# M-Gjerde/GaussianSplattingViewer

Measured on AMD Instinct MI355X. Metric: frames/sec + Msplats/sec, 1M Gaussians @ 1920×1080, 1/2/4/8 MI355X, higher is better.
Workload: dtype f32

## Files before the change

gaussiansplattingviewer_amd/csrc/api.hip:

```cpp
#include <algorithm>
#include <chrono>
#include <cstdio>
#include <cstdlib>
#include <cstring>
#include <mutex>
#include <string>
#include <vector>

#include "gsr.h"
#include "gsr_internal.h"

namespace {

thread_local std::string g_err;

int fail(int code, const std::string &msg) {
    g_err = msg;
    return code;
}

#define GSR_HIP(call, what)                                                                  \
    do {                                                                                     \
        hipError_t e_ = (call);                                                              \
        if (e_ != hipSuccess)                                                                \
// ... 70 lines not shown
    Buf<uint32_t> block_kept{bufs};
    Buf<uint32_t> color_ids{bufs};
    Buf<uint32_t> perm{bufs};
    Buf<uint32_t> ds_ctl{bufs};
    Buf<uint32_t> col_hist{bufs};
    Buf<uint32_t> tile_keys{bufs}, tile_vals{bufs}, tile_keys_alt{bufs}, tile_vals_alt{bufs};
    Buf<uint2> ranges_local{bufs};
    uint32_t *ranges_words() const { return reinterpret_cast<uint32_t *>(ranges_local.get()); }
    Buf<uint32_t> col_starts{bufs};
    Buf<uint32_t> blend_order{bufs};
    Buf<float> grad2d{bufs};
    Buf<int32_t> bwd_radii{bufs};
    Buf<float> cam_partials{bufs};
    Buf<uint64_t> det_slab{bufs}, det_partials{bufs};
    Buf<float> det_sums{bufs};
    Buf<uint8_t> det_marks{bufs};
    hipEvent_t ev_bwd[4] = {};
    bool bwd_timed = false;
    Buf<uint32_t> frame_words{bufs};
    uint32_t *list_n() const { return frame_words.get() + 1; }
    GsrHostWords *host_words = nullptr, *d_host_words = nullptr;
    uint32_t sort_tag = 0;
    uint32_t last_Dr = UINT32_MAX, last_D = UINT32_MAX;
    struct LastFrame {
        bool valid = false;
        int64_t K = 0;
        int64_t list = 0;
        bool tight = false;
        uint32_t gx = 0, gy = 0, rb = 0, re = 0;
        uint32_t *point_list = nullptr, *tiles_local = nullptr;
        bool packed = false;
        uint32_t id_mask = 0xFFFFFFFFu;
    } last;
    int cull = 1;
    int fast = 1;
    int depth_sort = -1;
    int tight = 1;
    int timing = 0;
    int64_t forwards = 0;
    int64_t timed_frames = 0;
    hipEvent_t ev[kTimingRing][kStages + 1] = {};
    hipEvent_t ev_color[kTimingRing][2] = {};
    int second_stream = 1;
    hipStream_t aux = nullptr;
    hipEvent_t fork = nullptr, join = nullptr;
    hipEvent_t compacted = nullptr;
    int graphs = 0;
    uint32_t ws_gen = 0;
    int64_t list_cap = 0;
    std::vector<GraphEntry> graph_cache;
    std::vector<hipGraphExec_t> graph_retired;
    uint64_t graph_clock = 0;
    int64_t graph_frames = 0, graph_records = 0, graph_overflows = 0;
};

namespace {

int order_stream(gsr_context *ctx, hipStream_t s) {
    if (ctx->ws_stream_set && s != ctx->ws_stream)
        GSR_HIP(hipDeviceSynchronize(), "hipDeviceSynchronize(stream switch)");
    ctx->ws_stream = s;
    ctx->ws_stream_set = true;
    return GSR_OK;
}

int grow(gsr_context *ctx, DevBuf &b, size_t bytes, hipStream_t s) {
// ... 60 lines not shown
}

template <typename Pred>
bool spin_on(const unsigned long long *word, Pred pred, uint64_t &value) {
    const auto t0 = std::chrono::steady_clock::now();
    for (uint32_t spin = 0;; ++spin) {
        value = __atomic_load_n(word, __ATOMIC_ACQUIRE);
        if (pred(value)) return true;
        if ((spin & 1023u) == 1023u && std::chrono::steady_clock::now() - t0 > kSpinLimit)
            return false;
    }
}

uint64_t host_word(const unsigned long long &word) {
    return __atomic_load_n(&word, __ATOMIC_ACQUIRE);
}

struct Frame {
    hipStream_t s;
    int64_t P;
    int W, H;
    uint32_t gx, gy, rb, re, rows_tiles;
    int y0, rows_out;
    uint64_t T_strip;
    bool dbg;
    int tmode;
    hipEvent_t *ev, *evc;
    bool compact_sort;
    bool msd_sort;
    bool main_publish;
    bool color_ids;
    bool colpairs;
    bool graph = false;
    int col_shift;
    uint32_t tag;
    bool wide_local;
    GsrPreprocessArgs pa;
    bool tight;
    int shading = GSR_SHADE_SPLAT;
    float *depth_map = nullptr, *inv_depth_map = nullptr;
    float *median_depth = nullptr;
    int32_t *median_id = nullptr;
    int feat_C = 0;
    const float *features = nullptr;
    float *feature_map = nullptr;
    bool no_blend = false;
    uint64_t K = 0;
    uint64_t KL = 0;
    uint32_t *point_list = nullptr, *tiles_local = nullptr;
    uint32_t id_mask = 0xFFFFFFFFu;
};

struct FrameRequest {
    int shading = GSR_SHADE_SPLAT;
    const gsr_depth_outputs *depth = nullptr;
    const gsr_surface_outputs *surface = nullptr;
    bool antialiasing = false;
    bool no_blend = false;
    const gsr_feature_outputs *feat = nullptr;
};

int stage_end(gsr_context *ctx, const Frame &f, int i) {
    if (f.tmode == 1 || (f.tmode == 2 && i >= 5))
        GSR_HIP(hipEventRecord(f.ev[i + 1], f.s), "hipEventRecord");
    if (f.dbg) {
        GSR_HIP(hipStreamSynchronize(f.s), std::string("stage ") + kStageNames[i]);
// ... 45 lines not shown
        f.feat_C = rq.feat->C, f.features = rq.feat->features, f.feature_map = rq.feat->feature_map;
    f.no_blend = rq.no_blend;
    f.P = P;
    f.W = W;
    f.H = H;
    f.gx = (uint32_t)((W + GSR_TILE_X - 1) / GSR_TILE_X);
    f.gy = (uint32_t)((H + GSR_TILE_Y - 1) / GSR_TILE_Y);
    if (f.gx > 0xFFFFu || f.gy > 0xFFFFu)
        return fail(GSR_E_INVALID, "gsr_forward: image larger than 65535 tiles per side");
    f.rb = 0;
    f.re = f.gy;
    if (st->tile_row_begin != 0 || st->tile_row_end != 0) {
        if (st->tile_row_begin < 0 || st->tile_row_end > (int)f.gy ||
            st->tile_row_begin >= st->tile_row_end)
            return fail(GSR_E_INVALID, "gsr_forward: bad tile row strip");
        f.rb = (uint32_t)st->tile_row_begin;
        f.re = (uint32_t)st->tile_row_end;
    }
    f.rows_tiles = f.re - f.rb;
    f.y0 = (int)(f.rb * GSR_TILE_Y);
    f.rows_out = std::min(H, (int)(f.re * GSR_TILE_Y)) - f.y0;
    f.T_strip = (uint64_t)f.gx * f.rows_tiles;
    f.dbg = st->debug != 0;
    f.ev = ctx->ev[ctx->timed_frames % kTimingRing];
    f.evc = ctx->ev_color[ctx->timed_frames % kTimingRing];
    f.tmode = ctx->timing == 1 ? 1 : (ctx->timing == 2 && ctx->forwards++ % 8 == 0) ? 2 : 0;

    const int ybits = f.rows_tiles > 1 ? bits_for(f.rows_tiles - 1) : 0;
    f.col_shift = 32 - ybits;
    f.colpairs = f.gx <= 256 && f.rows_tiles <= 256 &&
                 (f.col_shift == 32 || (uint64_t)P <= (1ull << f.col_shift));

    GSR_TRY(reserve_P(ctx, P, s));
    GSR_TRY(grow(ctx, ctx->ranges_local, (size_t)std::max<uint64_t>(f.T_strip, 1) * 8, s));
    if (f.colpairs) {
        GSR_TRY(grow(ctx, ctx->col_starts, 257 * 4, s));
        GSR_TRY(grow(ctx, ctx->blend_order,
                     (size_t)gsr_blend_order_groups((uint32_t)f.T_strip) * 4, s));
    }

    GsrPreprocessArgs &pa = f.pa;
    pa = GsrPreprocessArgs{};
    pa.P = P;
    pa.D = g->D;
    pa.M = g->M;
    pa.scale_modifier = g->scale_modifier;
    pa.means3D = g->means3D;
    pa.scales = g->scales;
    pa.rotations = g->rotations;
    pa.opacities = g->opacities;
    pa.shs = g->shs;
    pa.colors_precomp = g->colors_precomp;
    pa.cov3D_precomp = g->cov3D_precomp;
    pa.viewmatrix = st->viewmatrix;
    pa.projmatrix = st->projmatrix;
    pa.campos = st->campos;
    pa.tanfovx = st->tanfovx;
    pa.tanfovy = st->tanfovy;
    pa.focal_y = (float)H / (2.0f * st->tanfovy);
    pa.focal_x = (float)W / (2.0f * st->tanfovx);
    pa.W = W;
    pa.H = H;
    pa.grid_x = f.gx;
    pa.grid_y = f.gy;
    pa.row_begin = f.rb;
    pa.row_end = f.re;
    pa.prefiltered = st->prefiltered;
// ... 4 lines not shown
    pa.strip_skip = out->radii == nullptr ? 1 : 0;
    pa.records = ctx->records.get();
    pa.sort_keys = ctx->sort_keys.get();
    f.compact_sort = ctx->depth_sort < 0 ? (f.rows_tiles < f.gy && P >= kCompactP)
                                         : ctx->depth_sort == 1 || ctx->depth_sort == 3;
    pa.block_kept = f.compact_sort ? ctx->block_kept.get() : nullptr;
    f.msd_sort = ctx->depth_sort < 0
                     ? ctx->last_Dr <= (ctx->second_stream ? kMsdMaxD : kMsdMaxDOneStream)
                     : ctx->depth_sort >= 2;
    f.main_publish = f.msd_sort && !f.compact_sort;
    pa.strip_rect = ctx->strip_rect.get();
    f.tight = ctx->tight && f.colpairs && !out->n_contrib && f.rows_tiles == f.gy &&
              rq.shading != GSR_SHADE_BILLBOARD;
    pa.strip_rc = f.tight ? ctx->strip_rc.get() : nullptr;
    pa.block_pairs = ctx->pair_count.get();
    pa.host_words = ctx->d_host_words;
    pa.depths = out->depths;
    pa.means2D = out->means2D;
    pa.conic_opacity = out->conic_opacity;
    pa.rgb = out->rgb;
    pa.tiles_touched = out->tiles_touched;
    f.color_ids = f.compact_sort && gsr_color_ids_ok(pa);
    if (f.color_ids) GSR_TRY(grow(ctx, ctx->color_ids, (size_t)P * 4, s));
    f.tag = ++ctx->sort_tag;
    if (f.tag == 0) f.tag = ++ctx->sort_tag;
    pa.k_tag = f.tag;
    {
        const uint32_t crowd = (uint32_t)host_word(ctx->host_words->crowd);
        f.wide_local = crowd != 0u && f.tag - crowd <= kCrowdFrames;
    }
    return GSR_OK;
}

int launch_depth_sort(gsr_context *ctx, const Frame &f, int p0, int p1) {
    uint32_t *hist = ctx->hist.get(), *digit_total = ctx->digit_total.get();
    uint32_t *ctl = ctx->ds_ctl.get(), *perm = ctx->perm.get();
    uint2 *ds_a = ctx->ds_a.get(), *ds_b = ctx->ds_b.get();
    unsigned long long *host_D = &ctx->d_host_words->sort_D;
    hipError_t e;
    const int64_t nb = gsr_preprocess_blocks(f.P);
    const uint2 *keybits = reinterpret_cast<const uint2 *>(f.pa.block_pairs + nb);
    if (f.compact_sort) {
        if (f.msd_sort && p0 != 0) return GSR_OK;
        uint32_t *keys_c = ctx->ds_b_words(), *ids_c = keys_c + f.P;
        e = gsr_depth_sort_compacted(f.pa.sort_keys, f.P, f.pa.block_kept, keys_c, ids_c, ds_a,
                                     ds_b, perm, hist, digit_total, ctl, p0, p1, f.s, host_D,
                                     f.tag, f.color_ids ? ctx->color_ids.get() : nullptr,
                                     f.color_ids ? ctx->compacted : nullptr, f.msd_sort ? 1 : 0,
                                     f.msd_sort && !f.main_publish ? keybits : nullptr, nb);
    } else if (f.msd_sort) {
        if (p0 != 0) return GSR_OK;
        e = gsr_depth_sort_msd(f.pa.sort_keys, f.P, f.main_publish ? nullptr : keybits, nb,
                               ds_a, ds_b, perm, hist, digit_total, ctl, f.s,
                               f.graph ? nullptr : host_D, f.tag,
                               f.graph ? nullptr : &ctx->d_host_words->crowd,
                               f.graph ? 0 : f.wide_local);
    } else {
        e = gsr_depth_sort(f.pa.sort_keys, f.P, 1, ds_a, ds_b, perm, hist, digit_total, ctl, p0,
                           p1, f.s, f.graph ? nullptr : host_D, f.tag);
    }
    GSR_HIP(e, "depth sort launch");
    return GSR_OK;
}

constexpr int kColorWavesFull = 2, kColorWavesCompacted = 3, kColorWavesStrip = 4;
int color_waves_of(const Frame &f) {
// ... 107 lines not shown
                                       std::to_string(ctx->last_D) + ", sort " +
                                       std::to_string(ctl2[1]) + ")");
        if (!f.colpairs && scan_K[0] != f.K)
            return fail(GSR_E_HIP, "gsr_forward: pair count mismatch (preprocess " +
                                       std::to_string(f.K) + ", scan " +
                                       std::to_string(scan_K[0]) + ")");
    }
    int64_t want = (int64_t)f.KL;
    if (ctx->graphs && f.colpairs && want > ctx->list_cap) {
        ctx->list_cap = list_capacity(want, ctx->list_cap);
        want = ctx->list_cap;
    }
    return reserve_K(ctx, want, f.s);
}

uint32_t id_mask_of(int col_shift) {
    return col_shift < 32 ? (1u << col_shift) - 1u : 0xFFFFFFFFu;
}

int launch_col_binning(gsr_context *ctx, Frame &f, int64_t n, uint32_t *list_n) {
    uint32_t *tv = ctx->tile_vals.get(), *tv_alt = ctx->tile_vals_alt.get();
    uint32_t *col_starts = ctx->col_starts.get();
    if (n > 0)
        GSR_HIP(gsr_launch_col_pairs_scatter(ctx->perm.get(), ctx->rect_sorted.get(),
                                             f.tight ? ctx->rc_sorted.get() : nullptr, f.P,
                                             ctx->ds_ctl.get(), ctx->col_hist.get(),
                                             ctx->digit_total.get(), f.col_shift, tv_alt,
                                             col_starts, f.s,
                                             list_n ? (uint32_t)n : 0xFFFFFFFFu, list_n),
                "column scatter launch");
    std::swap(tv, tv_alt);
    GSR_TRY(stage_end(ctx, f, 3));
    const GsrTileStarts ts{col_starts, f.gx, f.rows_tiles, ctx->ranges_local.get(),
                           ctx->blend_order.get()};
    if (n > 0 && f.col_shift < 32)
        GSR_HIP(gsr_radix_sort_keys(&tv, &tv_alt, n, f.col_shift, 32, ctx->hist.get(),
                                    ctx->digit_total.get(), f.s, list_n, &ts),
                "tile sort launch");
    else
        GSR_HIP(gsr_launch_tile_runs(n, list_n, ts, f.s), "tile ranges launch");
    GSR_TRY(stage_end(ctx, f, 4));
    f.point_list = tv;
    f.tiles_local = nullptr;
    f.id_mask = id_mask_of(f.col_shift);
    return GSR_OK;
}

int launch_binning(gsr_context *ctx, Frame &f) {
    const int64_t K = (int64_t)f.KL;
    if (f.colpairs) return launch_col_binning(ctx, f, K, nullptr);
    const uint32_t *perm = ctx->perm.get(), *d_valid = ctx->ds_ctl.get();
    uint32_t *hist = ctx->hist.get(), *digit_total = ctx->digit_total.get();
    uint32_t *tk = ctx->tile_keys.get(), *tv = ctx->tile_vals.get();
    uint32_t *tk_alt = ctx->tile_keys_alt.get(), *tv_alt = ctx->tile_vals_alt.get();
    const int tbits = f.T_strip > 1 ? bits_for(f.T_strip - 1) : 0;
    const GsrRadixPlan plan = gsr_radix_plan(0, tbits);
    if (K > 0) {
        GSR_HIP(gsr_launch_scan_down(perm, ctx->rect_sorted.get(), ctx->partials.get(), f.P,
                                     d_valid, ctx->total.get(), ctx->bin.get(),
                                     ctx->chunk_first.get(), f.s),
                "scan_down launch");
        GSR_HIP(gsr_launch_dup_sort_pass(ctx->bin.get(), ctx->chunk_first.get(), K, f.gx,
                                         plan.n ? plan.shift[0] : 0, plan.n ? plan.nbits[0] : 0,
                                         hist, digit_total, tk_alt, tv_alt,
                                         ctx->ranges_local.get(), (uint32_t)f.T_strip, f.s),
                "duplicate launch");
        std::swap(tk, tk_alt);
// ... 51 lines not shown
    } else if (f.depth_map || f.inv_depth_map) {
        const GsrDepthArgs da{f.pa.sort_keys, f.depth_map, f.inv_depth_map};
        GSR_HIP(gsr_launch_blend_depth(ba, da, f.s), "depth blend launch");
    } else {
        GSR_HIP(gsr_launch_blend(ba, f.s), "blend launch");
    }
    if (f.feature_map)
        GSR_HIP(gsr_launch_blend_features(ba, f.features, f.feat_C, f.feature_map, f.s),
                "feature blend launch");
    return GSR_OK;
}

struct JoinGuard {
    hipStream_t s = nullptr;
    hipEvent_t join = nullptr;
    bool armed = false;
    ~JoinGuard() {
        if (armed) (void)hipStreamWaitEvent(s, join, 0);
    }
};

void finish_frame(gsr_context *ctx, const Frame &f, gsr_outputs *out) {
    out->num_rendered = (int64_t)f.K;
    gsr_context::LastFrame &l = ctx->last;
    l.K = (int64_t)f.K;
    l.list = (int64_t)f.KL;
    l.tight = f.tight;
    l.gx = f.gx, l.gy = f.gy, l.rb = f.rb, l.re = f.re;
    l.point_list = f.point_list;
    l.tiles_local = f.tiles_local;
    l.id_mask = f.id_mask;
    l.packed = f.colpairs && f.KL > 0;
    l.valid = true;
    if (f.tmode) ++ctx->timed_frames;
}

int frame_head(gsr_context *ctx, const Frame &f) {
    if (f.tmode == 1) GSR_HIP(hipEventRecord(f.ev[0], f.s), "hipEventRecord");
    GSR_HIP(gsr_launch_preprocess(f.pa, f.s), "preprocess launch");
    GSR_HIP(hipEventRecord(ctx->fork, f.s), "hipEventRecord(fork)");
    return stage_end(ctx, f, 0);
}

int frame_tail(gsr_context *ctx, const Frame &f, const gsr_raster_settings *st,
               gsr_outputs *out) {
    if (ctx->second_stream)
        GSR_HIP(hipStreamWaitEvent(f.s, ctx->join, 0), "hipStreamWaitEvent(join)");
    GSR_TRY(stage_end(ctx, f, 5));
    if (!f.no_blend) GSR_TRY(launch_blend(ctx, f, st, out));
    return stage_end(ctx, f, 6);
}


bool graph_eligible(const gsr_context *ctx, const Frame &f, const gsr_outputs *out) {
    return ctx->graphs && ctx->list_cap > 0 && f.colpairs && !f.dbg && f.tmode != 1 &&
           !f.compact_sort && !f.color_ids && !out->rgb && f.P > 0;
}

GraphKey graph_key(const gsr_context *ctx, const Frame &f) {
    GraphKey k;
    std::memset(&k, 0, sizeof(k));
    k.ws_gen = ctx->ws_gen;
    k.cap = ctx->list_cap;
    k.P = f.P;
    k.means3D = f.pa.means3D;
    k.shs = f.pa.shs;
    k.colors_precomp = f.pa.colors_precomp;
    k.D = f.pa.D;
    k.M = f.pa.M;
    k.W = f.W;
    k.H = f.H;
    k.gx = f.gx;
    k.gy = f.gy;
    k.rb = f.rb;
    k.re = f.re;
    k.col_shift = f.col_shift;
    k.color_waves = color_waves_of(f);
    k.msd = f.msd_sort;
    k.main_publish = f.main_publish;
    k.tight = f.tight;
    k.sh_vec4 = (uint8_t)f.pa.sh_vec4;
    return k;
}

GsrPreprocessArgs graph_args(const gsr_context *ctx, const GsrPreprocessArgs &a) {
    GsrPreprocessArgs g = a;
    g.campos = a.campos ? reinterpret_cast<const float *>(ctx->frame_words.get() + 4) : nullptr;
    g.viewmatrix = g.projmatrix = nullptr;
    g.scales = g.rotations = g.opacities = g.cov3D_precomp = nullptr;
    g.radii = nullptr;
    g.depths = g.means2D = g.conic_opacity = g.rgb = nullptr;
    g.tiles_touched = nullptr;
    g.k_tag = 0;
    g.frame_words = nullptr;
    return g;
}

void retire_graph(gsr_context *ctx, GraphEntry &e) {
    for (hipGraphExec_t *ge : {&e.sort, &e.bin, &e.aux}) {
        if (*ge) ctx->graph_retired.push_back(*ge);
        *ge = nullptr;
    }
}

int drain_retired(gsr_context *ctx, hipStream_t s, bool force) {
    if (ctx->graph_retired.empty() || (!force && ctx->graph_retired.size() < kGraphRetired))
        return GSR_OK;
    GSR_HIP(hipStreamSynchronize(s), "hipStreamSynchronize(graphs)");
    if (ctx->aux) GSR_HIP(hipStreamSynchronize(ctx->aux), "hipStreamSynchronize(graphs)");
    for (hipGraphExec_t ge : ctx->graph_retired) (void)hipGraphExecDestroy(ge);
    ctx->graph_retired.clear();
    return GSR_OK;
}

struct CaptureStream {
    hipStream_t s = nullptr;
    bool own = false;
    ~CaptureStream() {
        if (own && s) (void)hipStreamDestroy(s);
    }
};

template <typename Chain>
int record_chain(gsr_context *ctx, Chain chain, hipGraphExec_t *out) {
    CaptureStream capture;
    capture.s = ctx->aux;
    if (!capture.s) {
// ... 10 lines not shown
        if (graph) (void)hipGraphDestroy(graph);
        return rc;
    }
    GSR_HIP(e, "hipStreamEndCapture");
    const hipError_t ei = hipGraphInstantiate(out, graph, nullptr, nullptr, 0);
    (void)hipGraphDestroy(graph);
    GSR_HIP(ei, "hipGraphInstantiate");
    return GSR_OK;
}

Frame graph_frame(const gsr_context *ctx, const Frame &f) {
    Frame g = f;
    g.pa = graph_args(ctx, f.pa);
    g.tmode = 0;
    return g;
}

int chain_sort(gsr_context *ctx, Frame &g, hipStream_t cs) {
    g.s = cs;
    if (g.main_publish)
        GSR_HIP(gsr_launch_count_pairs(g.pa, cs, ctx->ds_ctl.get(), ctx->frame_words.get()),
                "pair count launch");
    return launch_depth_sort(ctx, g, 0, gsr_depth_sort_passes(32));
}

int chain_bin(gsr_context *ctx, Frame &g, hipStream_t cs) {
    g.s = cs;
    GSR_TRY(launch_scan(ctx, g));
    return launch_col_binning(ctx, g, ctx->list_cap, ctx->list_n());
}

int record_frame_graphs(gsr_context *ctx, const Frame &f, GraphEntry &e) {
    Frame g = graph_frame(ctx, f);
    const uint32_t *fw = ctx->frame_words.get();
    GSR_TRY(record_chain(ctx, [&](hipStream_t cs) { return chain_sort(ctx, g, cs); }, &e.sort));
    GSR_TRY(record_chain(ctx, [&](hipStream_t cs) { return chain_bin(ctx, g, cs); }, &e.bin));
    e.point_list = g.point_list;
    GSR_TRY(record_chain(ctx, [&](hipStream_t cs) { return aux_chain(ctx, g, cs, fw); }, &e.aux));
    ++ctx->graph_records;
    return GSR_OK;
}

int find_graphs(gsr_context *ctx, const Frame &f, GraphEntry **out) {
    const GraphKey key = graph_key(ctx, f);
    GraphEntry *hit = nullptr;
    for (auto it = ctx->graph_cache.begin(); it != ctx->graph_cache.end();) {
        if (it->key.ws_gen != ctx->ws_gen || it->key.cap != ctx->list_cap) {
            retire_graph(ctx, *it);
            it = ctx->graph_cache.erase(it);
            continue;
        }
        if (std::memcmp(&it->key, &key, sizeof(key)) == 0) hit = &*it;
        ++it;
    }
    if (!hit) {
        if (ctx->graph_cache.size() >= kGraphCache) {
            auto lru = std::min_element(ctx->graph_cache.begin(), ctx->graph_cache.end(),
                                        [](const GraphEntry &a, const GraphEntry &b) {
                                            return a.used < b.used;
                                        });
            retire_graph(ctx, *lru);
            ctx->graph_cache.erase(lru);
        }
        GraphEntry e;
        e.key = key;
        const int rc = record_frame_graphs(ctx, f, e);
        if (rc != GSR_OK) {
            retire_graph(ctx, e);
            return rc;
        }
        ctx->graph_cache.push_back(e);
        hit = &ctx->graph_cache.back();
    }
    hit->used = ++ctx->graph_clock;
    *out = hit;
    return GSR_OK;
}

constexpr int kOverflow = 1;
constexpr int kNoGraphs = 2;

int forward_graph(gsr_context *ctx, Frame &f, const gsr_raster_settings *st, gsr_outputs *out) {
    GraphEntry *e = nullptr;
    const bool replay = ctx->graphs == 1;
    if (replay && find_graphs(ctx, f, &e) != GSR_OK) return kNoGraphs;
    Frame g = graph_frame(ctx, f);
    uint32_t *fw = ctx->frame_words.get();
    hipStream_t s = f.s;
    f.pa.frame_words = fw;
    GSR_TRY(frame_head(ctx, f));
    if (replay) GSR_HIP(hipGraphLaunch(e->sort, s), "hipGraphLaunch(depth sort)");
    else GSR_TRY(chain_sort(ctx, g, s));
    const bool two = ctx->second_stream != 0;
    if (two) GSR_HIP(hipEventRecord(ctx->fork, s), "hipEventRecord(sorted)");
    if (two) GSR_HIP(hipStreamWaitEvent(ctx->aux, ctx->fork, 0), "hipStreamWaitEvent(fork)");
    if (replay) GSR_HIP(hipGraphLaunch(e->aux, two ? ctx->aux : s), "hipGraphLaunch(aux chain)");
    else GSR_TRY(aux_chain(ctx, g, two ? ctx->aux : s, fw));
    if (two) GSR_HIP(hipEventRecord(ctx->join, ctx->aux), "hipEventRecord(join)");
    if (replay) GSR_HIP(hipGraphLaunch(e->bin, s), "hipGraphLaunch(binning)");
    else GSR_TRY(chain_bin(ctx, g, s));
    f.point_list = replay ? e->point_list : g.point_list;
    f.tiles_local = nullptr;
    f.id_mask = id_mask_of(f.col_shift);
    GSR_TRY(frame_tail(ctx, f, st, out));
    ++ctx->graph_frames;
    GSR_TRY(read_K(ctx, f, publish_stream(ctx, f)));
    if ((int64_t)f.KL > ctx->list_cap) return kOverflow;
    finish_frame(ctx, f, out);
    return GSR_OK;
}

int forward(gsr_context *ctx, const gsr_gaussians *g, const gsr_raster_settings *st,
            gsr_outputs *out, hipStream_t s, const FrameRequest &rq) {
    Frame f;
    ctx->last.valid = false;
    GSR_TRY(setup_frame(ctx, g, st, out, s, rq, f));
    if (ctx->second_stream && !ctx->aux)
        GSR_HIP(hipStreamCreateWithPriority(&ctx->aux, hipStreamNonBlocking, 0),
                "hipStreamCreateWithPriority(second stream)");
    f.graph = graph_eligible(ctx, f, out);
    if (f.graph) {
        GSR_TRY(drain_retired(ctx, s, false));
        int rc = forward_graph(ctx, f, st, out);
        if (rc == kNoGraphs) {
            ctx->graphs = 2;
            rc = forward_graph(ctx, f, st, out);
        }
        if (rc != kOverflow) return rc;
        ++ctx->graph_overflows;
        ctx->list_cap = list_capacity((int64_t)f.KL, ctx->list_cap);
        GSR_TRY(reserve_K(ctx, ctx->list_cap, s));
        GSR_TRY(setup_frame(ctx, g, st, out, s, rq, f));
        f.graph = false;
    }

    if (f.P == 0) {
        GSR_HIP(hipMemsetAsync(out->color, 0, (size_t)3 * f.rows_out * f.W * sizeof(float), s),
                "hipMemsetAsync(color)");
        for (float *plane : {f.depth_map, f.inv_depth_map})
            if (plane)
                GSR_HIP(hipMemsetAsync(plane, 0, (size_t)f.rows_out * f.W * sizeof(float), s),
                        "hipMemsetAsync(depth plane)");
        if (f.median_depth)
            GSR_HIP(hipMemsetAsync(f.median_depth, 0, (size_t)f.rows_out * f.W * sizeof(float), s),
                    "hipMemsetAsync(median depth)");
        if (f.median_id)
            GSR_HIP(hipMemsetAsync(f.median_id, 0xFF, (size_t)f.rows_out * f.W * sizeof(int32_t), s),
                    "hipMemsetAsync(median id)");
        if (f.feature_map)
            GSR_HIP(hipMemsetAsync(f.feature_map, 0,
                                   (size_t)f.feat_C * f.rows_out * f.W * sizeof(float), s),
                    "hipMemsetAsync(feature map)");
        GSR_HIP(hipMemsetAsync(ctx->ranges_words(), 0, f.T_strip * 8, s), "hipMemsetAsync");
        f.K = f.KL = 0;
        f.tight = false;
        f.point_list = ctx->tile_vals.get();
        f.tiles_local = ctx->tile_keys.get();
        f.id_mask = 0xFFFFFFFFu;
        f.tmode = 0;
        finish_frame(ctx, f, out);
        return GSR_OK;
    }

    GSR_TRY(frame_head(ctx, f));
    if (f.main_publish)
        GSR_HIP(gsr_launch_count_pairs(f.pa, s, ctx->ds_ctl.get()), "pair count launch");
// ... 692 lines not shown
```

gaussiansplattingviewer_amd/csrc/blend_order.h:

```cpp
#pragma once

#include "gsr_internal.h"

namespace gsr {

constexpr uint32_t kGroupTiles = 4;

constexpr int kOrderBuckets = 1024;
__device__ __forceinline__ uint32_t order_key(const uint2 *ranges, uint32_t g, uint32_t n_tiles) {
    uint32_t n = 0;
    const uint32_t t0 = g * kGroupTiles;
#pragma unroll
    for (uint32_t i = 0; i < kGroupTiles; ++i)
        if (t0 + i < n_tiles) {
            const uint2 r = ranges[t0 + i];
            n += r.y - r.x;
        }
    const int k = (int)(__builtin_amdgcn_logf((float)n + 1.0f) * 32.0f);
    return (uint32_t)(kOrderBuckets - 1 - min(k, kOrderBuckets - 1));
}

template <int kThreads>
__device__ __forceinline__ void blend_order_block(const uint2 *ranges, uint32_t n_tiles,
                                                  uint32_t n_groups, uint32_t *order,
                                                  uint32_t *s_h, uint32_t *s_w) {
    constexpr int kPer = kOrderBuckets / kThreads;
    static_assert(kPer * kThreads == kOrderBuckets, "whole buckets per thread");
    const int tid = threadIdx.x;
    for (int i = tid; i < kOrderBuckets; i += kThreads) s_h[i] = 0u;
    __syncthreads();
    for (uint32_t g = tid; g < n_groups; g += kThreads)
        atomicAdd(&s_h[order_key(ranges, g, n_tiles)], 1u);
    __syncthreads();
    uint32_t c[kPer], sum = 0;
#pragma unroll
    for (int i = 0; i < kPer; ++i) sum += (c[i] = s_h[tid * kPer + i]);
    uint32_t x = sum;
    const int lane = tid & 63, w = tid >> 6;
#pragma unroll
    for (int o = 1; o < 64; o <<= 1) {
        const uint32_t y = __shfl_up(x, o);
        if (lane >= o) x += y;
    }
    if (lane == 63) s_w[w] = x;
    __syncthreads();
    uint32_t base = x - sum;
    for (int i = 0; i < w; ++i) base += s_w[i];
#pragma unroll
    for (int i = 0; i < kPer; ++i) {
        s_h[tid * kPer + i] = base;
        base += c[i];
    }
    __syncthreads();
    for (uint32_t g = tid; g < n_groups; g += kThreads)
        order[atomicAdd(&s_h[order_key(ranges, g, n_tiles)], 1u)] = g;
}

}
```

gaussiansplattingviewer_amd/csrc/gsr_internal.h:

```cpp
#pragma once
#include <hip/hip_runtime.h>
#include <stdint.h>

#pragma clang fp contract(off)

#define GSR_TILE_X 16
#define GSR_TILE_Y 16

namespace gsr {

struct alignas(16) SplatRecord {
    float4 a, b, c;
};

__device__ __forceinline__ int f2i_sat(float v) {
    if (!(v == v)) return 0;
    if (v >= 2147483648.0f) return 2147483647;
    if (v <= -2147483648.0f) return (-2147483647 - 1);
    return (int)v;
}

__device__ __forceinline__ float3 transform_point_4x3(float3 p, const float *M) {
    float3 r;
    r.x = M[0] * p.x + M[4] * p.y + M[8] * p.z + M[12];
// ... 230 lines not shown
    unsigned long long D;
    unsigned long long sort_D;
    unsigned long long K_spans;
    unsigned long long Dr;
    unsigned long long K_tag;
};
static_assert(sizeof(GsrHostWords) == 8 * sizeof(unsigned long long), "eight pinned words");

struct GsrPreprocessArgs {
    int64_t P;
    int D, M;
    float scale_modifier;
    const float *means3D, *scales, *rotations, *opacities, *shs, *colors_precomp, *cov3D_precomp;
    const float *viewmatrix, *projmatrix, *campos;
    float tanfovx, tanfovy, focal_x, focal_y;
    int W, H;
    uint32_t grid_x, grid_y, row_begin, row_end;
    int prefiltered;
    int sh_vec4, rot_vec4;
    int32_t *radii;
    int strip_skip;
    gsr::SplatRecord *records;
    uint32_t *sort_keys;
    uint32_t *block_kept;
    uint2 *strip_rect;
    uint4 *strip_rc;
    uint64_t *block_pairs;
    GsrHostWords *host_words;
    uint32_t k_tag;
    uint32_t *frame_words;
    float *depths, *means2D, *conic_opacity, *rgb;
    uint32_t *tiles_touched;
    int antialiasing;
};

inline int64_t gsr_preprocess_blocks(int64_t P) { return (P + 255) / 256; }
hipError_t gsr_launch_preprocess(const GsrPreprocessArgs &a, hipStream_t s);
hipError_t gsr_launch_color(const GsrPreprocessArgs &a, int waves_per_simd, hipStream_t s);
hipError_t gsr_color_setup();
bool gsr_color_ids_ok(const GsrPreprocessArgs &a);
hipError_t gsr_launch_color_ids(const GsrPreprocessArgs &a, const uint32_t *ids,
                                const uint32_t *d_n, int waves_per_simd, hipStream_t s);
hipError_t gsr_launch_count_pairs(const GsrPreprocessArgs &a, hipStream_t s,
                                  uint32_t *ds_ctl = nullptr, const uint32_t *d_tag = nullptr);
hipError_t gsr_launch_mark_visible(const float *means3D, int64_t P, const float *viewmatrix,
                                   uint8_t *visible, hipStream_t s);
hipError_t gsr_launch_view_depth_keys(const float *xyz, int64_t P, float v20, float v21, float v22,
                                      float v23, uint32_t *keys, float *depth_out, hipStream_t s);

int64_t gsr_radix_hist_words(int64_t n);
hipError_t gsr_radix_sort_pairs(uint32_t **keys, uint32_t **vals, uint32_t **keys_alt,
                                uint32_t **vals_alt, int64_t n, int begin_bit, int end_bit,
                                uint32_t *hist, uint32_t *digit_total, hipStream_t s,
                                int first_pass = 0);
struct GsrTileStarts {
    const uint32_t *col_starts;
    uint32_t gx, rows;
    uint2 *ranges;
    uint32_t *order;
};
hipError_t gsr_radix_sort_keys(uint32_t **keys, uint32_t **keys_alt, int64_t n, int begin_bit,
                               int end_bit, uint32_t *hist, uint32_t *digit_total, hipStream_t s,
                               const uint32_t *d_n = nullptr,
                               const GsrTileStarts *tile_starts = nullptr);
hipError_t gsr_launch_digit_scan(uint32_t *hist, int64_t nb, uint32_t *digit_total,
                                 hipStream_t s);
// ... 188 lines not shown
```

gaussiansplattingviewer_amd/csrc/preprocess.hip:

```cpp
#include <algorithm>

#include "gsr_internal.h"

using namespace gsr;

namespace {

__constant__ float kShC0 = 0.28209479177387814f;
__constant__ float kShC1 = 0.4886025119029199f;
__constant__ float kShC2[5] = {1.0925484305920792f, -1.0925484305920792f, 0.31539156525252005f,
                               -1.0925484305920792f, 0.5462742152960396f};
__constant__ float kShC3[7] = {-0.5900435899266435f, 2.890611442640554f, -0.4570457994644658f,
                               0.3731763325901154f, -0.4570457994644658f, 1.445305721320277f,
                               -0.5900435899266435f};

__device__ __forceinline__ float3 eval_sh(float3 pos, const float *campos, const float (&c)[48],
                                          int deg);

__device__ __forceinline__ float3 color_from_sh(float3 pos, const float *campos, const float *sh,
                                                int deg, bool vec_ok) {
    float c[48];
    const int ncoef = (deg + 1) * (deg + 1);
    if (vec_ok) {
        const float4 *v = reinterpret_cast<const float4 *>(sh);
        const int nvec = (ncoef * 3 + 3) >> 2;
        float4 rowv[12];
#pragma unroll
        for (int i = 0; i < 12; ++i) rowv[i] = v[i];
#pragma unroll
        for (int i = 0; i < 12; ++i) {
            float4 q = make_float4(0.f, 0.f, 0.f, 0.f);
            if (i < nvec) q = rowv[i];
            c[4 * i + 0] = q.x;
            c[4 * i + 1] = q.y;
// ... 287 lines not shown
                                                      rc.x0, rc.x1 - rc.x0, sy0, sy1 - sy0, cols);
                }
                if (strip_tiles) rec.c.x = cd.z;
                if (a.depths) a.depths[idx] = p_view.z;
                if (a.means2D) {
                    a.means2D[2 * idx] = px;
                    a.means2D[2 * idx + 1] = py;
                }
                if (a.conic_opacity)
                    reinterpret_cast<float4 *>(a.conic_opacity)[idx] =
                        make_float4(conic_a, conic_b, conic_c, opacity);
            }
        }
    }
    if (a.radii) a.radii[idx] = radius_out;
    a.strip_rect[idx] = strip_rect;
    if (a.strip_rc) a.strip_rc[idx] = make_uint4(strip_rect.x, strip_rect.y, cols.x, cols.y);
    tight_out =
        (strip_rect.x && a.strip_rc && span_coded(strip_rect)) ? strip_tiles_tight : strip_tiles;
    a.sort_keys[idx] = key;
    key_out = key;
    if (a.tiles_touched) a.tiles_touched[idx] = strip_tiles;
    return strip_tiles;
}

struct SkipSmem {
    float v[12][256];
    uint32_t idx[256];
    uint32_t wcount[4];
};

template <bool kSkip, bool kAA>
__device__ __forceinline__ void preprocess_block(const GsrPreprocessArgs &a) {
    const int64_t idx = (int64_t)blockIdx.x * blockDim.x + threadIdx.x;
    uint32_t key = 0xFFFFFFFFu;
    uint32_t pairs = 0u, tight = 0u;
    if (!kSkip) {
        if (idx < a.P) pairs = back_one<kAA>(a, idx, front_one(a, idx), key, tight);
    } else {
        __shared__ SkipSmem sk;
        const int lane = threadIdx.x & 63, w = threadIdx.x >> 6;
        bool reach = false;
        Front f;
        if (idx < a.P) {
            f = front_one(a, idx);
            reach = f.in_frustum &&
                    strip_reach(a, f.p_view, f.cov3d, ndc2pix(f.p_proj_y, a.H));
            if (!reach) none_one(a, idx);
        }
        const uint64_t bal = __ballot(reach);
        if (lane == 0) sk.wcount[w] = (uint32_t)__popcll(bal);
        __syncthreads();
        uint32_t base = 0, n = 0;
#pragma unroll
        for (int i = 0; i < 4; ++i) {
            base += i < w ? sk.wcount[i] : 0u;
            n += sk.wcount[i];
        }
        if (reach) {
            const uint64_t lt = lane == 0 ? 0ull : (~0ull >> (64 - lane));
            const uint32_t slot = base + (uint32_t)__popcll(bal & lt);
            sk.v[0][slot] = f.p_view.x;
            sk.v[1][slot] = f.p_view.y;
            sk.v[2][slot] = f.p_view.z;
            sk.v[3][slot] = f.p_proj_x;
            sk.v[4][slot] = f.p_proj_y;
#pragma unroll
// ... 2 lines not shown
            sk.idx[slot] = (uint32_t)idx;
        }
        __syncthreads();
        if (threadIdx.x < n) {
            const uint32_t t = threadIdx.x;
            Front g;
            g.p_view = make_float3(sk.v[0][t], sk.v[1][t], sk.v[2][t]);
            g.p_proj_x = sk.v[3][t];
            g.p_proj_y = sk.v[4][t];
#pragma unroll
            for (int i = 0; i < 6; ++i) g.cov3d[i] = sk.v[5 + i][t];
            g.opacity = sk.v[11][t];
            g.in_frustum = true;
            pairs = back_one<kAA>(a, (int64_t)sk.idx[t], g, key, tight);
        }
    }
    const bool kept = pairs != 0u;
    uint32_t v = pairs, mx = kept ? key : 0u, mn = kept ? key : 0xFFFFFFFFu;
#pragma unroll
    for (int off = 32; off > 0; off >>= 1) {
        v += __shfl_xor(v, off);
        tight += __shfl_xor(tight, off);
        mx = max(mx, (uint32_t)__shfl_xor(mx, off));
        mn = min(mn, (uint32_t)__shfl_xor(mn, off));
    }
    __shared__ uint32_t s_red[5][4];
    const uint32_t c = a.block_kept ? (uint32_t)__popcll(__ballot(kept)) : 0u;
    if ((threadIdx.x & 63) == 0) {
        const int w = threadIdx.x >> 6;
        s_red[0][w] = v, s_red[1][w] = mx, s_red[2][w] = mn, s_red[3][w] = c, s_red[4][w] = tight;
    }
    __syncthreads();
    if (threadIdx.x == 0) {
        if (a.frame_words && blockIdx.x == 0) {
            a.frame_words[0] = a.k_tag;
            if (a.campos) {
                a.frame_words[4] = __float_as_uint(a.campos[0]);
                a.frame_words[5] = __float_as_uint(a.campos[1]);
                a.frame_words[6] = __float_as_uint(a.campos[2]);
            }
        }
        a.block_pairs[blockIdx.x] =
            ((uint64_t)(s_red[4][0] + s_red[4][1] + s_red[4][2] + s_red[4][3]) << 32) |
            (s_red[0][0] + s_red[0][1] + s_red[0][2] + s_red[0][3]);
        reinterpret_cast<uint2 *>(a.block_pairs + gridDim.x)[blockIdx.x] =
            make_uint2(max(max(s_red[1][0], s_red[1][1]), max(s_red[1][2], s_red[1][3])),
                       min(min(s_red[2][0], s_red[2][1]), min(s_red[2][2], s_red[2][3])));
        if (a.block_kept) a.block_kept[blockIdx.x] = s_red[3][0] + s_red[3][1] + s_red[3][2] + s_red[3][3];
    }
}

template <bool kSkip>
__global__ __launch_bounds__(256) void k_preprocess(const GsrPreprocessArgs a) {
    preprocess_block<kSkip, false>(a);
}
template <bool kSkip>
__global__ __launch_bounds__(256) void k_preprocess_aa(const GsrPreprocessArgs a) {
    preprocess_block<kSkip, true>(a);
}

constexpr int kPubThreads = 1024, kPubWaves = kPubThreads / 64;
__global__ __launch_bounds__(kPubThreads) void k_publish_K(const unsigned long long *__restrict__ cnt,
                                                           const uint2 *__restrict__ keybits,
                                                           int64_t n, GsrHostWords *host,
                                                           uint32_t k_tag, uint32_t *ds_ctl,
                                                           const uint32_t *d_tag) {
    __shared__ unsigned long long s_w[kPubWaves], s_wt[kPubWaves];
    __shared__ uint32_t s_max[kPubWaves], s_min[kPubWaves];
    unsigned long long v = 0, vt = 0;
    uint32_t mx = 0u, mn = 0xFFFFFFFFu;
    constexpr int kU = 8;
    for (int64_t i0 = threadIdx.x; i0 < n; i0 += kU * kPubThreads) {
        unsigned long long c[kU];
        uint2 kb[kU];
#pragma unroll
        for (int u = 0; u < kU; ++u) {
            const int64_t i = i0 + (int64_t)u * kPubThreads;
            c[u] = i < n ? cnt[i] : 0ull;
            kb[u] = i < n ? keybits[i] : make_uint2(0u, 0xFFFFFFFFu);
        }
#pragma unroll
// ... 115 lines not shown
                                     a.means3D[3 * idx + 2]);
        store_color(a, idx, eval_sh3_stream(p, a.campos,
                                            reinterpret_cast<const float4 *>(a.shs) + idx * 12));
    }
    if (a.P < 0) s_occupancy_cap[threadIdx.x] = 0u;
}

__global__ __launch_bounds__(256) void k_mark_visible(const float *__restrict__ means3D,
                                                      int64_t P, const float *viewmatrix,
                                                      uint8_t *visible) {
    const int64_t idx = (int64_t)blockIdx.x * blockDim.x + threadIdx.x;
    if (idx >= P) return;
    const float3 p = make_float3(means3D[3 * idx], means3D[3 * idx + 1], means3D[3 * idx + 2]);
    visible[idx] = transform_point_4x3(p, viewmatrix).z > 0.2f ? 1 : 0;
}

__global__ __launch_bounds__(256) void k_view_depth_keys(const float *__restrict__ xyz, int64_t P,
                                                         float v20, float v21, float v22, float v23,
                                                         uint32_t *keys, float *depth_out) {
    const int64_t idx = (int64_t)blockIdx.x * blockDim.x + threadIdx.x;
    if (idx >= P) return;
    const float x = xyz[3 * idx], y = xyz[3 * idx + 1], z = xyz[3 * idx + 2];
    const float d = __builtin_fmaf(v22, z, __builtin_fmaf(v20, x, v21 * y)) + v23;
    keys[idx] = float_sort_key(d);
    if (depth_out) depth_out[idx] = d;
}

inline unsigned grid_for(int64_t n) { return (unsigned)gsr_preprocess_blocks(n); }

}

hipError_t gsr_launch_preprocess(const GsrPreprocessArgs &a, hipStream_t s) {
    if (a.P == 0) return hipSuccess;
    if (a.antialiasing && a.strip_skip)
        hipLaunchKernelGGL(k_preprocess_aa<true>, dim3(grid_for(a.P)), dim3(256), 0, s, a);
    else if (a.antialiasing)
        hipLaunchKernelGGL(k_preprocess_aa<false>, dim3(grid_for(a.P)), dim3(256), 0, s, a);
    else if (a.strip_skip)
        hipLaunchKernelGGL(k_preprocess<true>, dim3(grid_for(a.P)), dim3(256), 0, s, a);
    else
        hipLaunchKernelGGL(k_preprocess<false>, dim3(grid_for(a.P)), dim3(256), 0, s, a);
    return hipGetLastError();
}

hipError_t gsr_launch_color(const GsrPreprocessArgs &a, int waves_per_simd, hipStream_t s) {
    if (a.P == 0) return hipSuccess;
    const unsigned g0 = grid_for(a.P);
    if (!a.sh_vec4 || a.colors_precomp || a.D != 3) {
        hipLaunchKernelGGL(k_color_generic, dim3(g0), dim3(256), 0, s, a);
        return hipGetLastError();
    }
    const size_t lds = (waves_per_simd >= 1 && waves_per_simd < 8)
                           ? (size_t)(160 * 1024 / waves_per_simd) & ~(size_t)1023
                           : 0;
    hipLaunchKernelGGL(k_color, dim3(g0), dim3(256), lds, s, a);
    return hipGetLastError();
}

hipError_t gsr_color_setup() {
    return hipFuncSetAttribute(reinterpret_cast<const void *>(&k_color),
                               hipFuncAttributeMaxDynamicSharedMemorySize, 160 * 1024);
}

bool gsr_color_ids_ok(const GsrPreprocessArgs &a) {
    return a.sh_vec4 && !a.colors_precomp && a.D == 3 && !a.rgb;
}

hipError_t gsr_launch_color_ids(const GsrPreprocessArgs &a, const uint32_t *ids,
                                const uint32_t *d_n, int waves_per_simd, hipStream_t s) {
    if (a.P == 0) return hipSuccess;
    if (!gsr_color_ids_ok(a)) return hipErrorInvalidValue;
    size_t lds = 0;
    if (waves_per_simd >= 3 && waves_per_simd < 8)
        lds = (size_t)(160 * 1024 / waves_per_simd) & ~(size_t)1023;
// ... 31 lines not shown
```

gaussiansplattingviewer_amd/csrc/radix_sort.hip:

```cpp
#include <algorithm>

#include "blend_order.h"
#include "radix_tile.h"

using namespace gsr;

namespace {

constexpr int kBlock = 256;
constexpr int kRadix = kRadixBins;

struct RsCount {
    int64_t n_host;
    const uint32_t *d_n;
};

__device__ __forceinline__ int64_t live_count(const uint32_t *d_n, int64_t n_cap) {
    if (!d_n) return n_cap;
    const int64_t n = (int64_t)*d_n;
    return n <= n_cap ? n : 0;
}

template <int kW, int kIt, int kTiles>
__global__ __launch_bounds__(kW * 64) void k_rs_upsweep(const uint32_t *__restrict__ keys,
// ... 229 lines not shown

static int64_t hist_stride(int64_t nb) { return (nb + 3) & ~(int64_t)3; }
constexpr int64_t kQuadTiles = 4096;

int64_t gsr_radix_hist_words(int64_t n) {
    const int64_t nb = (n + kST - 1) / kST;
    return (nb < 1 ? 4 : hist_stride(nb)) * kRadix;
}

static void rts_pass(const uint32_t *k, const uint32_t *v, uint32_t *ko, uint32_t *vo, int64_t n,
                     int shift, int nbits, uint32_t *hist, uint32_t *digit_total, hipStream_t s,
                     const uint32_t *d_n = nullptr, const GsrTileStarts *tile_starts = nullptr) {
    const int64_t nb = (n + kST - 1) / kST;
    if (nb == 0) return;
    const int64_t stride = hist_stride(nb);
    const uint32_t mask = (1u << nbits) - 1u;
    if (nb >= kQuadTiles)
        hipLaunchKernelGGL((k_rs_upsweep<kSW, kSIt, 4>),
                           dim3(xcd_run_grid((nb + 3) / 4)), dim3(kSW * 64), 0, s,
                           k, n, shift, mask, hist, stride, d_n);
    else
        hipLaunchKernelGGL((k_rs_upsweep<kSW, kSIt, 1>), dim3(xcd_run_grid(nb)),
                           dim3(kSW * 64), 0, s, k, n, shift, mask, hist, stride, d_n);
    hipLaunchKernelGGL(k_rs_scan, dim3(kRadix), dim3(kBlock), 0, s, hist, stride, digit_total,
                       RsCount{nb, d_n}, kST);
    const GsrTileStarts ts = tile_starts ? *tile_starts : GsrTileStarts{};
    const dim3 down_grid(xcd_run_grid(nb) + (ts.gx ? tile_start_blocks(ts.gx) : 0u));
    if (v)
        hipLaunchKernelGGL((k_rs_downsweep<kSW, kSIt, true>), down_grid, dim3(kSW * 64), 0, s, k,
                           v, ko, vo, n, shift, nbits, hist, digit_total, stride, d_n, ts);
    else
        hipLaunchKernelGGL((k_rs_downsweep<kSW, kSIt, false>), down_grid, dim3(kSW * 64), 0, s,
                           k, v, ko, vo, n, shift, nbits, hist, digit_total, stride, d_n, ts);
    if (ts.gx)
        hipLaunchKernelGGL(k_blend_order, dim3(1), dim3(kOrderThreads), 0, s, ts);
}

hipError_t gsr_radix_sort_pairs(uint32_t **keys, uint32_t **vals, uint32_t **keys_alt,
                                uint32_t **vals_alt, int64_t n, int begin_bit, int end_bit,
                                uint32_t *hist, uint32_t *digit_total, hipStream_t s,
                                int first_pass) {
    if (n <= 1) return hipSuccess;
    const GsrRadixPlan plan = gsr_radix_plan(begin_bit, end_bit);
    for (int p = first_pass; p < plan.n; ++p) {
        rts_pass(*keys, *vals, *keys_alt, *vals_alt, n, plan.shift[p], plan.nbits[p], hist,
                 digit_total, s);
        std::swap(*keys, *keys_alt);
        std::swap(*vals, *vals_alt);
    }
    return hipGetLastError();
}

hipError_t gsr_radix_sort_keys(uint32_t **keys, uint32_t **keys_alt, int64_t n, int begin_bit,
                               int end_bit, uint32_t *hist, uint32_t *digit_total, hipStream_t s,
                               const uint32_t *d_n, const GsrTileStarts *tile_starts) {
    const GsrRadixPlan plan = gsr_radix_plan(begin_bit, end_bit);
    if (tile_starts && (plan.n != 1 || n < 1 || tile_starts->gx < 1 ||
                        tile_starts->gx > (uint32_t)kRadix || tile_starts->rows > (uint32_t)kRadix))
        return hipErrorInvalidValue;
    if (n <= 1 && !d_n && !tile_starts) return hipSuccess;
    for (int p = 0; p < plan.n; ++p) {
        rts_pass(*keys, nullptr, *keys_alt, nullptr, n, plan.shift[p], plan.nbits[p], hist,
                 digit_total, s, d_n, tile_starts);
        std::swap(*keys, *keys_alt);
    }
    return hipGetLastError();
}

namespace {

__global__ __launch_bounds__(kBlock) void k_tile_runs(int64_t n_cap,
                                                      const uint32_t *__restrict__ d_n,
                                                      const GsrTileStarts ts) {
    __shared__ uint32_t s_h[kOrderBuckets];
    __shared__ uint32_t s_w[kBlock / 64];
    const int64_t n = live_count(d_n, n_cap);
    const uint32_t n_tiles = ts.gx * ts.rows;
    for (uint32_t t = threadIdx.x; t < n_tiles; t += kBlock) {
        uint2 out = make_uint2(0u, 0u);
        if (n > 0) {
            const uint32_t B0 = ts.col_starts[t], B1 = ts.col_starts[t + 1];
            if (B0 < B1 && (int64_t)B1 <= n) out = make_uint2(B0, B1);
        }
        ts.ranges[t] = out;
    }
    __syncthreads();
    blend_order_block<kBlock>(ts.ranges, n_tiles, (n_tiles + kGroupTiles - 1) / kGroupTiles,
                              ts.order, s_h, s_w);
}

}

hipError_t gsr_launch_tile_runs(int64_t n, const uint32_t *d_n, const GsrTileStarts &ts,
                                hipStream_t s) {
    if (ts.gx == 0 || ts.rows == 0) return hipSuccess;
    if (n > 0 && (ts.rows != 1 || ts.gx > (uint32_t)kRadix)) return hipErrorInvalidValue;
    hipLaunchKernelGGL(k_tile_runs, dim3(1), dim3(kBlock), 0, s, n, d_n, ts);
    return hipGetLastError();
}
```

Measured before the change: 4561.

## Compute blend order from previous frame's tile ranges inside preprocess kernel

Removes the single-block k_blend_order launch from the serial binning chain. Instead, an extra block in the preprocess kernel builds the tile blend order from the previous frame's per-tile ranges, so the order lags one frame behind but overlaps with preprocessing. The order_key loads are also vectorized with uint4 and the histogram loops are unrolled by four, which needs ranges padded to a multiple of four. The carry only happens when geometry and buffers are unchanged and is disabled under graph replay. The risk is a stale load-balancing order after view changes.

```diff
diff --git a/gaussiansplattingviewer_amd/csrc/api.hip b/gaussiansplattingviewer_amd/csrc/api.hip
--- a/gaussiansplattingviewer_amd/csrc/api.hip
+++ b/gaussiansplattingviewer_amd/csrc/api.hip
@@ -126,6 +126,13 @@
         bool packed = false;
         uint32_t id_mask = 0xFFFFFFFFu;
     } last;
+    struct OrderCarry {
+        bool ok = false;
+        uint32_t gx = 0, rows = 0;
+        uint64_t T_strip = 0;
+        const void *ranges = nullptr, *order = nullptr;
+        size_t ranges_cap = 0, order_cap = 0;
+    } carry;
     int cull = 1;
     int fast = 1;
     int depth_sort = -1;
@@ -252,6 +259,7 @@
     bool color_ids;
     bool colpairs;
     bool graph = false;
+    bool carry = false;
     int col_shift;
     uint32_t tag;
     bool wide_local;
@@ -363,7 +371,7 @@
                  (f.col_shift == 32 || (uint64_t)P <= (1ull << f.col_shift));
 
     GSR_TRY(reserve_P(ctx, P, s));
-    GSR_TRY(grow(ctx, ctx->ranges_local, (size_t)std::max<uint64_t>(f.T_strip, 1) * 8, s));
+    GSR_TRY(grow(ctx, ctx->ranges_local, (size_t)((std::max<uint64_t>(f.T_strip, 1) + 3) & ~3ull) * 8, s));
     if (f.colpairs) {
         GSR_TRY(grow(ctx, ctx->col_starts, 257 * 4, s));
         GSR_TRY(grow(ctx, ctx->blend_order,
@@ -434,6 +442,25 @@
     return GSR_OK;
 }
 
+void drop_carry(Frame &f) {
+    f.carry = false;
+    f.pa.prev_ranges = nullptr;
+    f.pa.order = nullptr;
+    f.pa.order_tiles = 0;
+}
+void carry_order(const gsr_context *ctx, const gsr_context::OrderCarry &prev, Frame &f) {
+    drop_carry(f);
+    if (!(prev.ok && f.colpairs && f.P > 0 && prev.gx == f.gx && prev.rows == f.rows_tiles &&
+          prev.T_strip == f.T_strip && prev.ranges == ctx->ranges_local.p &&
+          prev.ranges_cap == ctx->ranges_local.cap && prev.order == ctx->blend_order.p &&
+          prev.order_cap == ctx->blend_order.cap))
+        return;
+    f.carry = true;
+    f.pa.prev_ranges = ctx->ranges_local.get();
+    f.pa.order = ctx->blend_order.get();
+    f.pa.order_tiles = (uint32_t)f.T_strip;
+}
+
 int launch_depth_sort(gsr_context *ctx, const Frame &f, int p0, int p1) {
     uint32_t *hist = ctx->hist.get(), *digit_total = ctx->digit_total.get();
     uint32_t *ctl = ctx->ds_ctl.get(), *perm = ctx->perm.get();
@@ -607,7 +634,7 @@
     std::swap(tv, tv_alt);
     GSR_TRY(stage_end(ctx, f, 3));
     const GsrTileStarts ts{col_starts, f.gx, f.rows_tiles, ctx->ranges_local.get(),
-                           ctx->blend_order.get()};
+                           f.carry ? nullptr : ctx->blend_order.get()};
     if (n > 0 && f.col_shift < 32)
         GSR_HIP(gsr_radix_sort_keys(&tv, &tv_alt, n, f.col_shift, 32, ctx->hist.get(),
                                     ctx->digit_total.get(), f.s, list_n, &ts),
@@ -725,6 +752,11 @@
     l.id_mask = f.id_mask;
     l.packed = f.colpairs && f.KL > 0;
     l.valid = true;
+    gsr_context::OrderCarry &c = ctx->carry;
+    c.ok = f.colpairs && f.P > 0;
+    c.gx = f.gx, c.rows = f.rows_tiles, c.T_strip = f.T_strip;
+    c.ranges = ctx->ranges_local.p, c.ranges_cap = ctx->ranges_local.cap;
+    c.order = ctx->blend_order.p, c.order_cap = ctx->blend_order.cap;
     if (f.tmode) ++ctx->timed_frames;
 }
 
@@ -786,6 +818,7 @@
     g.tiles_touched = nullptr;
     g.k_tag = 0;
     g.frame_words = nullptr;
+    g.prev_ranges = nullptr, g.order = nullptr, g.order_tiles = 0;
     return g;
 }
 
@@ -862,6 +895,7 @@
 
 int record_frame_graphs(gsr_context *ctx, const Frame &f, GraphEntry &e) {
     Frame g = graph_frame(ctx, f);
+    g.carry = false;
     const uint32_t *fw = ctx->frame_words.get();
     GSR_TRY(record_chain(ctx, [&](hipStream_t cs) { return chain_sort(ctx, g, cs); }, &e.sort));
     GSR_TRY(record_chain(ctx, [&](hipStream_t cs) { return chain_bin(ctx, g, cs); }, &e.bin));
@@ -914,6 +948,7 @@
     GraphEntry *e = nullptr;
     const bool replay = ctx->graphs == 1;
     if (replay && find_graphs(ctx, f, &e) != GSR_OK) return kNoGraphs;
+    if (replay) drop_carry(f);
     Frame g = graph_frame(ctx, f);
     uint32_t *fw = ctx->frame_words.get();
     hipStream_t s = f.s;
@@ -944,7 +979,10 @@
             gsr_outputs *out, hipStream_t s, const FrameRequest &rq) {
     Frame f;
     ctx->last.valid = false;
+    const gsr_context::OrderCarry prev = ctx->carry;
+    ctx->carry.ok = false;
     GSR_TRY(setup_frame(ctx, g, st, out, s, rq, f));
+    carry_order(ctx, prev, f);
     if (ctx->second_stream && !ctx->aux)
         GSR_HIP(hipStreamCreateWithPriority(&ctx->aux, hipStreamNonBlocking, 0),
                 "hipStreamCreateWithPriority(second stream)");
@@ -962,6 +1000,7 @@
         GSR_TRY(reserve_K(ctx, ctx->list_cap, s));
         GSR_TRY(setup_frame(ctx, g, st, out, s, rq, f));
         f.graph = false;
+        drop_carry(f);
     }
 
     if (f.P == 0) {
diff --git a/gaussiansplattingviewer_amd/csrc/blend_order.h b/gaussiansplattingviewer_amd/csrc/blend_order.h
--- a/gaussiansplattingviewer_amd/csrc/blend_order.h
+++ b/gaussiansplattingviewer_amd/csrc/blend_order.h
@@ -8,17 +8,19 @@
 
 constexpr int kOrderBuckets = 1024;
 __device__ __forceinline__ uint32_t order_key(const uint2 *ranges, uint32_t g, uint32_t n_tiles) {
-    uint32_t n = 0;
+    static_assert(kGroupTiles == 4, "two uint4 per group");
     const uint32_t t0 = g * kGroupTiles;
-#pragma unroll
-    for (uint32_t i = 0; i < kGroupTiles; ++i)
-        if (t0 + i < n_tiles) {
-            const uint2 r = ranges[t0 + i];
-            n += r.y - r.x;
-        }
+    const uint4 *p = reinterpret_cast<const uint4 *>(ranges + t0);
+    const uint4 a = p[0], b = p[1];
+    uint32_t n = a.y - a.x;
+    n += t0 + 1 < n_tiles ? a.w - a.z : 0u;
+    n += t0 + 2 < n_tiles ? b.y - b.x : 0u;
+    n += t0 + 3 < n_tiles ? b.w - b.z : 0u;
     const int k = (int)(__builtin_amdgcn_logf((float)n + 1.0f) * 32.0f);
     return (uint32_t)(kOrderBuckets - 1 - min(k, kOrderBuckets - 1));
 }
+
+constexpr int kOrderUnroll = 4;
 
 template <int kThreads>
 __device__ __forceinline__ void blend_order_block(const uint2 *ranges, uint32_t n_tiles,
@@ -29,8 +31,15 @@
     const int tid = threadIdx.x;
     for (int i = tid; i < kOrderBuckets; i += kThreads) s_h[i] = 0u;
     __syncthreads();
-    for (uint32_t g = tid; g < n_groups; g += kThreads)
-        atomicAdd(&s_h[order_key(ranges, g, n_tiles)], 1u);
+    for (uint32_t g0 = tid; g0 < n_groups; g0 += kOrderUnroll * kThreads) {
+        uint32_t key[kOrderUnroll];
+#pragma unroll
+        for (int u = 0; u < kOrderUnroll; ++u)
+            key[u] = order_key(ranges, min(g0 + u * kThreads, n_groups - 1u), n_tiles);
+#pragma unroll
+        for (int u = 0; u < kOrderUnroll; ++u)
+            if (g0 + u * kThreads < n_groups) atomicAdd(&s_h[key[u]], 1u);
+    }
     __syncthreads();
     uint32_t c[kPer], sum = 0;
 #pragma unroll
@@ -52,8 +61,16 @@
         base += c[i];
     }
     __syncthreads();
-    for (uint32_t g = tid; g < n_groups; g += kThreads)
-        order[atomicAdd(&s_h[order_key(ranges, g, n_tiles)], 1u)] = g;
+    for (uint32_t g0 = tid; g0 < n_groups; g0 += kOrderUnroll * kThreads) {
+        uint32_t key[kOrderUnroll];
+#pragma unroll
+        for (int u = 0; u < kOrderUnroll; ++u)
+            key[u] = order_key(ranges, min(g0 + u * kThreads, n_groups - 1u), n_tiles);
+#pragma unroll
+        for (int u = 0; u < kOrderUnroll; ++u)
+            if (g0 + u * kThreads < n_groups)
+                order[atomicAdd(&s_h[key[u]], 1u)] = g0 + u * kThreads;
+    }
 }
 
 }
diff --git a/gaussiansplattingviewer_amd/csrc/gsr_internal.h b/gaussiansplattingviewer_amd/csrc/gsr_internal.h
--- a/gaussiansplattingviewer_amd/csrc/gsr_internal.h
+++ b/gaussiansplattingviewer_amd/csrc/gsr_internal.h
@@ -286,6 +286,9 @@
     float *depths, *means2D, *conic_opacity, *rgb;
     uint32_t *tiles_touched;
     int antialiasing;
+    const uint2 *prev_ranges;
+    uint32_t *order;
+    uint32_t order_tiles;
 };
 
 inline int64_t gsr_preprocess_blocks(int64_t P) { return (P + 255) / 256; }
diff --git a/gaussiansplattingviewer_amd/csrc/preprocess.hip b/gaussiansplattingviewer_amd/csrc/preprocess.hip
--- a/gaussiansplattingviewer_amd/csrc/preprocess.hip
+++ b/gaussiansplattingviewer_amd/csrc/preprocess.hip
@@ -1,5 +1,6 @@
 #include <algorithm>
 
+#include "blend_order.h"
 #include "gsr_internal.h"
 
 using namespace gsr;
@@ -353,7 +354,19 @@
 
 template <bool kSkip, bool kAA>
 __device__ __forceinline__ void preprocess_block(const GsrPreprocessArgs &a) {
-    const int64_t idx = (int64_t)blockIdx.x * blockDim.x + threadIdx.x;
+    uint32_t blk = blockIdx.x, n_blocks = gridDim.x;
+    if (a.prev_ranges) {
+        if (blk == 0) {
+            __shared__ uint32_t s_oh[kOrderBuckets];
+            __shared__ uint32_t s_ow[4];
+            blend_order_block<256>(a.prev_ranges, a.order_tiles,
+                                   (a.order_tiles + kGroupTiles - 1) / kGroupTiles, a.order, s_oh,
+                                   s_ow);
+            return;
+        }
+        --blk, --n_blocks;
+    }
+    const int64_t idx = (int64_t)blk * blockDim.x + threadIdx.x;
     uint32_t key = 0xFFFFFFFFu;
     uint32_t pairs = 0u, tight = 0u;
     if (!kSkip) {
@@ -422,7 +435,7 @@
     }
     __syncthreads();
     if (threadIdx.x == 0) {
-        if (a.frame_words && blockIdx.x == 0) {
+        if (a.frame_words && blk == 0) {
             a.frame_words[0] = a.k_tag;
             if (a.campos) {
                 a.frame_words[4] = __float_as_uint(a.campos[0]);
@@ -430,13 +443,13 @@
                 a.frame_words[6] = __float_as_uint(a.campos[2]);
             }
         }
-        a.block_pairs[blockIdx.x] =
+        a.block_pairs[blk] =
             ((uint64_t)(s_red[4][0] + s_red[4][1] + s_red[4][2] + s_red[4][3]) << 32) |
             (s_red[0][0] + s_red[0][1] + s_red[0][2] + s_red[0][3]);
-        reinterpret_cast<uint2 *>(a.block_pairs + gridDim.x)[blockIdx.x] =
+        reinterpret_cast<uint2 *>(a.block_pairs + n_blocks)[blk] =
             make_uint2(max(max(s_red[1][0], s_red[1][1]), max(s_red[1][2], s_red[1][3])),
                        min(min(s_red[2][0], s_red[2][1]), min(s_red[2][2], s_red[2][3])));
-        if (a.block_kept) a.block_kept[blockIdx.x] = s_red[3][0] + s_red[3][1] + s_red[3][2] + s_red[3][3];
+        if (a.block_kept) a.block_kept[blk] = s_red[3][0] + s_red[3][1] + s_red[3][2] + s_red[3][3];
     }
 }
 
@@ -618,14 +631,16 @@
 
 hipError_t gsr_launch_preprocess(const GsrPreprocessArgs &a, hipStream_t s) {
     if (a.P == 0) return hipSuccess;
+    if (a.prev_ranges && (!a.order || a.order_tiles == 0)) return hipErrorInvalidValue;
+    const dim3 grid(grid_for(a.P) + (a.prev_ranges ? 1u : 0u));
     if (a.antialiasing && a.strip_skip)
-        hipLaunchKernelGGL(k_preprocess_aa<true>, dim3(grid_for(a.P)), dim3(256), 0, s, a);
+        hipLaunchKernelGGL(k_preprocess_aa<true>, grid, dim3(256), 0, s, a);
     else if (a.antialiasing)
-        hipLaunchKernelGGL(k_preprocess_aa<false>, dim3(grid_for(a.P)), dim3(256), 0, s, a);
+        hipLaunchKernelGGL(k_preprocess_aa<false>, grid, dim3(256), 0, s, a);
     else if (a.strip_skip)
-        hipLaunchKernelGGL(k_preprocess<true>, dim3(grid_for(a.P)), dim3(256), 0, s, a);
+        hipLaunchKernelGGL(k_preprocess<true>, grid, dim3(256), 0, s, a);
     else
-        hipLaunchKernelGGL(k_preprocess<false>, dim3(grid_for(a.P)), dim3(256), 0, s, a);
+        hipLaunchKernelGGL(k_preprocess<false>, grid, dim3(256), 0, s, a);
     return hipGetLastError();
 }
 
diff --git a/gaussiansplattingviewer_amd/csrc/radix_sort.hip b/gaussiansplattingviewer_amd/csrc/radix_sort.hip
--- a/gaussiansplattingviewer_amd/csrc/radix_sort.hip
+++ b/gaussiansplattingviewer_amd/csrc/radix_sort.hip
@@ -285,7 +285,7 @@
     else
         hipLaunchKernelGGL((k_rs_downsweep<kSW, kSIt, false>), down_grid, dim3(kSW * 64), 0, s,
                            k, v, ko, vo, n, shift, nbits, hist, digit_total, stride, d_n, ts);
-    if (ts.gx)
+    if (ts.gx && ts.order)
         hipLaunchKernelGGL(k_blend_order, dim3(1), dim3(kOrderThreads), 0, s, ts);
 }
 
@@ -337,6 +337,7 @@
         }
         ts.ranges[t] = out;
     }
+    if (!ts.order) return;
     __syncthreads();
     blend_order_block<kBlock>(ts.ranges, n_tiles, (n_tiles + kGroupTiles - 1) / kGroupTiles,
                               ts.order, s_h, s_w);
```

Result: no change. 4579 (median of 4 runs) (+0.4%).
